# tp7/Sushi

Measured on AMD Instinct MI355X. Metric: subtitle events/sec (matchTemplate+argmax) + max |shift err| vs cv2, 1/2/4/8 GPU, higher is better.
Workload: dtype f32; 1 GPU; BASELINE configs[2] (the north_star target's configuration): 3000 events, 120-min 12000 Hz float32 src/dst, +-120 s window (P=2880001 positions, patterns U[1,5] s), explicit centres; the whole job every step; global_events=3000, sample_type=float32, hard_events=0, events_with_a_planted_answer=3000, method=TM_SQDIFF_NORMED+argmin (what wav.py:185-186 does; see SURVEY F1), kernel_variant=2

## Files before the change

### sushi_amd/csrc/plan_core.hpp

```cpp
#ifndef SUSHI_PLAN_CORE_HPP
#define SUSHI_PLAN_CORE_HPP

#include <limits.h>
#include <math.h>
#include <stdint.h>
#include <stdio.h>
#include <stdlib.h>
#include <string.h>

#include <algorithm>
#include <cmath>
#include <vector>

#include "sushi_geometry.hpp"

namespace sushi {

inline int64_t cand_capacity(int64_t pairs) {
    const int64_t want = pairs * 64;
    return want < (1 << 16) ? (1 << 16) : (want > (1 << 24) ? (1 << 24) : want);
}

struct WsLayout { size_t tspec, y, cand, pair_lb, pairmap, tconst, tiles, candbuf, dummy, slb, acc, plist, slist, citems,
                  tspec_low, ylow, audit_mark, slist2, dense_search, ditems, votes, total; };
// ... 197 lines not shown
            sb.item_count[kern] = mac_items(s, lay, a0, b0, kern, plan.items, &sb.chunk_group[kern]);
        }
        subs.push_back(sb);
        a0 = b0;
    }
    return SUSHI_HIP_OK;
}

inline bool complete_whole_cut(const std::vector<SearchDesc>& descs, Plan& plan) {
    Plan tmp;
    std::vector<SubBatch> subs;
    if (build_plan(descs, search_layouts(descs), plan.ws_whole, tmp, subs) != SUSHI_HIP_OK || subs.empty()) return false;
    if (subs.size() > plan.subs.size()) return false;
    if (tmp.order.size() > plan.order.size() - plan.whole_order_first || tmp.items.size() > plan.whole_items_room) return false;
    std::copy(tmp.order.begin(), tmp.order.end(), plan.order.begin() + (ptrdiff_t)plan.whole_order_first);
    std::copy(tmp.items.begin(), tmp.items.end(), plan.items.begin() + (ptrdiff_t)plan.whole_items_first);
    for (SubBatch& sb : subs) {
        sb.order_first += (int)plan.whole_order_first;
        for (int kern = 0; kern < 2; ++kern) sb.item_first[kern] += (int)(plan.whole_items_first / (1 + MAC_SPW));
    }
    plan.subs_whole.swap(subs);
    plan.whole_pending = false;
    return true;
}

struct BatchLayout { size_t desc, keys, flags, viol, flag_list, subc, tnorm, counters, order, items, ws, total; };

constexpr size_t SUBC_BYTES = 256;
constexpr int SUBC_SCOUNT = 8;
static_assert(sizeof(SubCounters) <= SUBC_SCOUNT * sizeof(int), "the scount words lie behind the SubCounters");
enum ScountSlot {
    SC_SLIST = 0,
    SC_CITEMS = 1,
    SC_ANY_DENSE = 4,
    SC_SLIST2 = 5,
    SC_DENSE_LISTED = 6,
    SC_LIST3 = 7,
    SC_WORDS = 8
};
static_assert((SUBC_SCOUNT + SC_WORDS) * sizeof(int) <= SUBC_BYTES, "the scount words fit the sub-batch's block");
inline BatchLayout batch_layout(int n, int path, size_t n_order_ints, size_t n_item_ints, size_t ws_bytes, size_t n_subs, int64_t total_segs) {
    BatchLayout b;
    size_t o = 0;
    b.desc = o; o += align_up((size_t)n * sizeof(SearchDesc), 256);
    b.order = o; o += path == SUSHI_HIP_PATH_FFT ? align_up(n_order_ints * sizeof(int32_t), 256) : 0;
    b.items = o; o += path == SUSHI_HIP_PATH_FFT ? align_up(n_item_ints * sizeof(int32_t), 256) : 0;
    b.keys = o; o += align_up((size_t)2 * n * sizeof(unsigned long long), 256);
    b.flags = o; o += align_up((size_t)n * sizeof(int), 256);
    b.viol = o; o += align_up((size_t)n * sizeof(int), 256);
    b.flag_list = o; o += align_up((size_t)n * sizeof(int), 256);
    b.subc = o; o += std::max<size_t>(n_subs, 1) * SUBC_BYTES;
    b.tnorm = o; o += align_up((size_t)total_segs * sizeof(float), 256);
    b.counters = o; o += align_up(sizeof(RunCounters), 256);
    b.ws = o; o += path == SUSHI_HIP_PATH_FFT ? align_up(ws_bytes, 256) : 0;
    b.total = o;
    return b;
}

inline int make_descs(const SushiHipRequest* req, int n, int tp, std::vector<SearchDesc>& out, int64_t* n_tiles,
                      int64_t dst_n = INT64_MAX, int64_t src_n = INT64_MAX) {
    out.resize(n);
    int64_t tiles = 0, pairs = 0, segs = 0;
    for (int k = 0; k < n; ++k) {
        const SushiHipRequest& r = req[k];
        if (!request_fits(r, dst_n, src_n)) return SUSHI_HIP_EINVAL;
        SearchDesc d;
// ... 93 lines not shown
```

### sushi_amd/csrc/run_policy.hpp

```cpp
#ifndef SUSHI_RUN_POLICY_HPP
#define SUSHI_RUN_POLICY_HPP

#include <stdint.h>
#include <string.h>

#include <algorithm>

#include "sushi_geometry.hpp"

namespace sushi {

enum RunKind { RUN_ARGMIN, RUN_THRESHOLD, RUN_BEST };

struct Learnt {
    int band = -1;
    int band_decided_method = -1;
    int band_votes[2] = {0, 0};
    int suspended = 0;
    unsigned suspended_at = 0;
    unsigned long long last_transformed = 0;
    void forget() { *this = Learnt(); }
};

struct LastRun {
    RunKind kind = RUN_ARGMIN;
    int band = -1;
    bool whole_cut = false;
    bool suspended = false;
    int64_t direct_pairs = 0;
    bool ran = false;
};

constexpr double SUSPEND_LEFT_SHARE = 0.75;
constexpr unsigned LOOK_AGAIN_MASK = 63u;
constexpr int64_t EXCLUDE_FROM_PAIRS = 3000, EXCLUDE_PAIRS_PER_SEARCH = 2;
constexpr double BAND_VOTE_SHARE = 0.75;
constexpr int64_t DIRECT_SLOTS_MIN = 4096, DIRECT_USUAL_PART = 8;
constexpr int64_t DIRECT_FIRST_RUN_PART = 2;

inline void absorb_counts(Learnt& l, int exclusion, unsigned run_seq, unsigned long long transformed, unsigned long long audited,
                          int64_t plan_pairs) {
// ... 20 lines not shown
    return exclusion == SUSHI_HIP_EXCLUDE_ALWAYS || exclusion == SUSHI_HIP_EXCLUDE_BAND || exclusion == SUSHI_HIP_EXCLUDE_WHOLE ||
           (exclusion == SUSHI_HIP_EXCLUDE_AUTO && !suspended && pairs > EXCLUDE_FROM_PAIRS + EXCLUDE_PAIRS_PER_SEARCH * (int64_t)n_sub);
}

inline bool listed_run_excludes(int exclusion) { return exclusion != SUSHI_HIP_EXCLUDE_NEVER; }

inline bool form_chosen(int exclusion) { return exclusion == SUSHI_HIP_EXCLUDE_BAND || exclusion == SUSHI_HIP_EXCLUDE_WHOLE; }
inline bool vote_due(const Learnt& l, int exclusion, int method) {
    return !form_chosen(exclusion) && (l.band < 0 || l.band_decided_method != method);
}
inline void decide_form(Learnt& l, int method, int looked_at, int with_room) {
    l.band_votes[0] = looked_at; l.band_votes[1] = with_room;
    l.band = l.band_votes[0] > 0 && (double)l.band_votes[1] >= BAND_VOTE_SHARE * (double)l.band_votes[0] ? 1 : 0;
    l.band_decided_method = method;
}
inline int exclusion_form(const Learnt& l, int exclusion) {
    return !form_chosen(exclusion) ? l.band : exclusion == SUSHI_HIP_EXCLUDE_BAND ? 1 : 0;
}

inline int64_t direct_slots(unsigned long long last_transformed, int64_t pairs, int64_t plan_pairs) {
    int64_t direct64 = std::min<int64_t>(pairs, std::max<int64_t>(DIRECT_SLOTS_MIN, pairs / DIRECT_USUAL_PART));
    if ((double)last_transformed * (double)pairs > (double)direct64 * (double)plan_pairs) direct64 = pairs;
    else if (last_transformed == 0) direct64 = std::min<int64_t>(pairs, std::max<int64_t>(DIRECT_SLOTS_MIN, pairs / DIRECT_FIRST_RUN_PART));
    return direct64;
}

enum { PILOT_ROWS_BY_SEARCH = 0, PILOT_ROWS_LIST = 1 };
inline int pilot_rows_route(const char* setting) {
    if (!setting || !*setting || !strcmp(setting, "search")) return PILOT_ROWS_BY_SEARCH;
    return !strcmp(setting, "list") ? PILOT_ROWS_LIST : -1;
}
inline bool pilot_rows_by_search(int route) { return route != PILOT_ROWS_LIST; }

inline void begin_run(LastRun& last, RunKind kind) {
    last = LastRun();
    last.kind = kind; last.ran = true;
}

inline void report_last_run(const LastRun& last, const Learnt& l, const RunCounters& c, SushiHipBatchDiag* diag) {
    const bool argmin = last.kind == RUN_ARGMIN;
    diag->pairs_transformed = (int64_t)c.pairs_transformed + last.direct_pairs;
    diag->band = last.band;
    diag->suspended = argmin && last.suspended ? 1 : 0;
    diag->band_votes[0] = argmin ? l.band_votes[0] : 0; diag->band_votes[1] = argmin ? l.band_votes[1] : 0;
    diag->second_look_audited = argmin ? (int64_t)c.second_look_audited : 0;
}

}
#endif
```

### sushi_amd/csrc/sushi_fft.hip

```cpp

#include <hip/hip_runtime.h>
#include <stdint.h>
#include <float.h>
#include <limits.h>
#include <stdio.h>
#include <stdlib.h>
#include <string.h>

#include <algorithm>
#include <cmath>
#include <memory>
#include <mutex>
#include <new>
#include <string>
#include <type_traits>
#include <vector>

#include "../../include/sushi_hip.h"
#include "sushi_common.hpp"
#include "sushi_internal.hpp"
#include "fft_core.hpp"
#include "mac_core.hpp"
#include "plan_core.hpp"
#include "batch_core.hpp"
// ... 41 lines not shown
        return base + (size_t)k * WORDS;
    }
    void give(unsigned long long* p) {
        if (!p) return;
        std::lock_guard<std::mutex> g(mu);
        free_list.push_back((int)((p - base) / WORDS));
    }
};
static HostSlots g_host_slots;

struct LanePool {
    static constexpr int MAX_DEVICES = 16;
    std::mutex mu;
    hipStream_t st[MAX_DEVICES][MAX_LANES] = {};
    hipStream_t get(int lane) {
        int dev = 0;
        if (hipGetDevice(&dev) != hipSuccess || dev < 0 || dev >= MAX_DEVICES) return nullptr;
        std::lock_guard<std::mutex> g(mu);
        if (!st[dev][lane] && hipStreamCreateWithFlags(&st[dev][lane], hipStreamNonBlocking) != hipSuccess) st[dev][lane] = nullptr;
        return st[dev][lane];
    }
};
static LanePool g_lane_pool;

struct SushiHipBatch {
    const SushiHipStream* dst = nullptr;
    const SushiHipStream* src = nullptr;
    int n = 0, path = 0, variant = 0, method = SUSHI_HIP_METHOD_SQDIFF_NORMED, exclusion = SUSHI_HIP_EXCLUDE_AUTO;
    Learnt learnt;
    LastRun last;
    unsigned run_seq = 0;
    int audit_every = 2;
    int pilot_rows = PILOT_ROWS_BY_SEARCH;
    int bound_model = SUSHI_HIP_BOUND_WORST_CASE;
    BoundFault fault;
    unsigned long long* host_stats = nullptr;
    hipEvent_t stats_ready = nullptr;
    bool stats_pending = false;
    int32_t* packed_out = nullptr;
    int32_t* early_out = nullptr;
    BatchPlanState states[2];
    BatchPlanState *now = &states[0], *spare = &states[1];
    bool planned = false;
    size_t mem_bytes = 0, ws_cap = 0;
    char* mem = nullptr;
    hipStream_t last_stream = nullptr;
    hipEvent_t uploaded = nullptr;
    hipStream_t lane_stream[MAX_LANES] = {};
    hipEvent_t lane_done[MAX_LANES] = {};
    hipEvent_t fork = nullptr;
    void forget_learnt() { learnt.forget(); last = LastRun(); }
    ~SushiHipBatch() {
        for (int l = 1; l < MAX_LANES; ++l) {
            if (lane_stream[l]) (void)hipStreamSynchronize(lane_stream[l]);
            if (lane_done[l]) (void)hipEventDestroy(lane_done[l]);
        }
        if (fork) (void)hipEventDestroy(fork);
        if (uploaded) { (void)hipEventSynchronize(uploaded); (void)hipEventDestroy(uploaded); }
        if (stats_pending && stats_ready) (void)hipEventSynchronize(stats_ready);
        if (stats_ready) (void)hipEventDestroy(stats_ready);
        g_host_slots.give(host_stats);
    }
};

static SubView last_sub(const SushiHipBatch* b) {
    const std::vector<SubBatch>& subs = b->last.whole_cut ? b->now->plan.subs_whole : b->now->plan.subs;
// ... 174 lines not shown
        ma.n_items = sb.item_count[kern];
        const int chunks = (low ? LROWE : ROWE) / MAC_BW;
        ma.chunk_group = std::min(sb.chunk_group[kern], chunks / 8);
        const dim3 grid((unsigned)chunks * (unsigned)ma.n_items);
        auto go = [&](auto row) {
            if (kern == 0) hipLaunchKernelGGL(mac_kernel<decltype(row)::value>, grid, dim3(MAC_THREADS), 0, st, ma);
            else hipLaunchKernelGGL(mac_long_kernel<decltype(row)::value>, grid, dim3(MAC_THREADS), 0, st, ma);
        };
        if (low) go(std::integral_constant<int, LROWE>()); else go(std::integral_constant<int, ROWE>());
        if (launch_ok() != SUSHI_HIP_OK) return SUSHI_HIP_ELAUNCH;
    }
    return SUSHI_HIP_OK;
}

static int launch_mac_list(const RunCtx& c, const SubView& v, hipStream_t st, const int* list, const int* count, int n_list,
                           const int* dense_search, int long_only) {
    MacListArgs la;
    la.dense_search = dense_search; la.long_only = long_only;
    la.spec = (const uint4*)c.dst->spec; la.spec_blocks = c.dst->blocks; la.tspec = (const uint4*)v.tspec; la.y = v.y;
    la.searches = c.searches + v.sb.a0; la.tconst = v.tconst; la.pairmap = v.pairmap; la.list = list; la.count = count;
    la.n_list = n_list; la.sub_first_seg = v.sb.first_seg; la.sub_first_pair = v.sb.first_pair;
    const int64_t want = (int64_t)n_list * MACL_PARTS;
    hipLaunchKernelGGL(mac_list_kernel, dim3((unsigned)std::min<int64_t>(want, 256 * 32)), dim3(MACL_THREADS), 0, st, la);
    return launch_ok();
}

static int launch_mac_rows(const RunCtx& c, const SubView& v, hipStream_t st, const BoundArgs& ba, const int mode) {
    const SubBatch& sb = v.sb;
    MacRowsArgs ra;
    ra.spec = (const uint4*)c.dst->spec; ra.spec_blocks = c.dst->blocks; ra.tspec = (const uint4*)v.tspec; ra.y = v.y;
    ra.searches = c.searches + sb.a0; ra.tconst = v.tconst; ra.mark = ba.audit_mark; ra.n_sub = v.n_sub;
    ra.sub_first_seg = sb.first_seg; ra.sub_first_pair = sb.first_pair; ra.dense_search = v.dense_search;
    ra.plist = ba.plist; ra.first_search = ba.first_search; ra.audit_seq = ba.audit_seq; ra.audit_every = ba.audit_every;
    const int64_t rows_want = (int64_t)v.n_sub * MACL_PARTS;
    const dim3 grid0((unsigned)std::min<int64_t>(rows_want, 256 * 32)), grid1((unsigned)std::min<int64_t>(rows_want, 256 * 16));
    auto go = [&](auto m) {
        if (sb.item_count[0] > 0) hipLaunchKernelGGL((mac_rows_kernel<0, decltype(m)::value>), grid0, dim3(MACL_THREADS), 0, st, ra);
        if (sb.item_count[1] > 0) hipLaunchKernelGGL((mac_rows_kernel<1, decltype(m)::value>), grid1, dim3(MACL_THREADS), 0, st, ra);
    };
    if (mode == ROWS_FIRST) go(std::integral_constant<int, ROWS_FIRST>());
    else if (mode == ROWS_REST) go(std::integral_constant<int, ROWS_REST>());
    else go(std::integral_constant<int, ROWS_MARKED>());
    return launch_ok();
}

static int launch_ifft(const RunCtx& c, const IfftArgs& x, unsigned grid, hipStream_t st) {
    const bool strided = x.count && !x.list_direct;
    return launch_method(c.method, [&](auto m) {
        if (strided) hipLaunchKernelGGL(ifft_list_kernel<decltype(m)::value>, dim3(grid), dim3(FT), 0, st, x);
        else hipLaunchKernelGGL(ifft_kernel<decltype(m)::value>, dim3(grid), dim3(FT), 0, st, x);
    });
}

static int bound_pairs(const RunCtx& c, const SubView& v, hipStream_t st, const int band, BoundArgs& ba) {
    const SubBatch& sb = v.sb;
    ba = bound_args(c, v);
    ba.band = band;
    ba.y = band ? (const uint2*)v.ylow : (const uint2*)v.y;
    if (!band && hipMemsetAsync(ba.acc, 0, (size_t)sb.pairs * 2 * sizeof(float), st) != hipSuccess) return SUSHI_HIP_ELAUNCH;
    const int per_pair = band ? 1 : 16;
    const int64_t want = (sb.pairs * per_pair + BOUND_THREADS / 64 - 1) / (BOUND_THREADS / 64);
    const unsigned grid = (unsigned)std::min<int64_t>(want, 256 * (band ? 3 * (c.lanes > 1 ? 2 : 4) : 4));
    auto go = [&](auto energies) {
        if (band) hipLaunchKernelGGL(bound_low_kernel<decltype(energies)::value>, dim3(grid), dim3(BOUND_THREADS), 0, st, ba);
        else hipLaunchKernelGGL(bound_kernel<decltype(energies)::value>, dim3(grid), dim3(BOUND_THREADS), 0, st, ba);
    };
    if (ba.worst_case) go(std::false_type()); else go(std::true_type());
    if (launch_ok() != SUSHI_HIP_OK || launch_slb(c, v, ba, st) != SUSHI_HIP_OK) return SUSHI_HIP_ELAUNCH;
    if (c.b->fault.period > 0) return launch_bound_fault(c, v, st);
    return SUSHI_HIP_OK;
}

static int second_look(const RunCtx& c, const SubView& v, hipStream_t st, BoundArgs& ba) {
    ba.list = ba.slist; ba.list_count = ba.scount;
    ba.list2 = v.slist2; ba.list2_count = v.n_slist2;
    hipLaunchKernelGGL(bound_low_exact_kernel, dim3(256 * 4), dim3(BLE_T), 0, st, ba);
    if (launch_ok() != SUSHI_HIP_OK) return SUSHI_HIP_ELAUNCH;
    if (launch_method(c.method, [&](auto m) { hipLaunchKernelGGL(slb_list_kernel<decltype(m)::value>, dim3(256 * 2), dim3(256), 0, st, ba); }) !=
        SUSHI_HIP_OK)
        return SUSHI_HIP_ELAUNCH;
    if (c.b->fault.period > 0 && launch_bound_fault(c, v, st) != SUSHI_HIP_OK) return SUSHI_HIP_ELAUNCH;
    hipLaunchKernelGGL(survivor2_kernel, dim3(256), dim3(256), 0, st, ba);
    return launch_ok();
}

static int exclude_pairs(const RunCtx& c, const SubView& v, hipStream_t st, const int band, IfftArgs& ip, hipEvent_t& t0) {
    const SubBatch& sb = v.sb;
    BoundArgs ba;
    if (bound_pairs(c, v, st, band, ba) != SUSHI_HIP_OK) return SUSHI_HIP_ELAUNCH;
    prof_end(c.pc, t0, SUSHI_HIP_STAGE_BOUND, st);
    t0 = prof_begin(c.pc, st);
    hipLaunchKernelGGL(pilot_kernel, dim3((unsigned)v.n_sub), dim3(64), 0, st, ba);
    if (launch_ok() != SUSHI_HIP_OK) return SUSHI_HIP_ELAUNCH;
    ip.slb = ba.slb; ip.audit_mark = nullptr;
    ip.order = ba.plist; ip.count = nullptr;
    const bool by_search = pilot_rows_by_search(c.b->pilot_rows);
    if (band && by_search && launch_mac_rows(c, v, st, ba, ROWS_FIRST) != SUSHI_HIP_OK) return SUSHI_HIP_ELAUNCH;
    if (band && launch_mac_list(c, v, st, ba.plist, nullptr, v.n_sub, nullptr, by_search ? 1 : 0) != SUSHI_HIP_OK) return SUSHI_HIP_ELAUNCH;
    if (launch_ifft(c, ip, (unsigned)v.n_sub, st) != SUSHI_HIP_OK) return SUSHI_HIP_ELAUNCH;
    hipLaunchKernelGGL(survivor_kernel, dim3((unsigned)((sb.pairs + 255) / 256)), dim3(256), 0, st, ba);
    if (launch_ok() != SUSHI_HIP_OK) return SUSHI_HIP_ELAUNCH;
    ip.order = ba.slist; ip.count = ba.scount; ip.audit_mark = ba.audit_mark;
    if (!band) return SUSHI_HIP_OK;
    if (second_look(c, v, st, ba) != SUSHI_HIP_OK) return SUSHI_HIP_ELAUNCH;
    ip.order = ba.list2; ip.count = ba.list2_count;
    hipLaunchKernelGGL(dense_search_kernel, dim3((unsigned)v.n_sub), dim3(64), 0, st, ba, v.dense_search, v.n_dense_listed);
    const size_t second = (size_t)(sb.item_first[1] - sb.item_first[0]) * (1 + MAC_SPW);
    hipLaunchKernelGGL(dense_repack_kernel, dim3(2), dim3(REPACK_THREADS), 0, st, v.items, sb.item_count[0], v.items + second,
                       sb.item_count[1], v.dense_search, v.n_sub, v.ditems, v.ditems + second, v.n_dense_listed, (int)(sb.pairs / 8),
                       v.any_dense);
    if (launch_ok() != SUSHI_HIP_OK) return SUSHI_HIP_ELAUNCH;
    if (launch_mac_rows(c, v, st, ba, by_search ? ROWS_REST : ROWS_MARKED) != SUSHI_HIP_OK) return SUSHI_HIP_ELAUNCH;
    if (sb.long_patterns && launch_mac_list(c, v, st, ba.list2, ba.list2_count, (int)sb.pairs, v.dense_search, 1) != SUSHI_HIP_OK) return SUSHI_HIP_ELAUNCH;
    return launch_mac(c, v, st, false, v.any_dense, v.ditems);
}

static int transform_listed(const RunCtx& c, const SubView& v, hipStream_t st, IfftArgs ip) {
    const SubBatch& sb = v.sb;
    const SushiHipBatch* b = c.b;
    const unsigned direct = (unsigned)direct_slots(b->learnt.last_transformed, sb.pairs, b->now->plan.pairs);
    ip.list_first = 0; ip.list_direct = 1;
    if (launch_ifft(c, ip, direct, st) != SUSHI_HIP_OK) return SUSHI_HIP_ELAUNCH;
    if ((int64_t)direct >= sb.pairs) return SUSHI_HIP_OK;
    ip.list_first = (int)direct; ip.list_direct = 0;
    return launch_ifft(c, ip, (unsigned)std::min<int64_t>(sb.pairs - direct, 1024), st);
}

static int stage_refine(const RunCtx& c, const SubView& v, hipStream_t st) {
    hipEvent_t t0 = prof_begin(c.pc, st);
    RefineParams rp;
    rp.r = c.r; rp.searches = c.searches; rp.first_search = v.sb.a0; rp.n_sub = v.n_sub; rp.sub_first_pair = v.sb.first_pair;
    rp.cand = v.cand; rp.pair_lb = v.pair_lb; rp.gkeys = c.gkeys; rp.keys = c.keys; rp.flags = c.flags; rp.flag_list = c.flag_list + v.sb.a0;
    rp.sub = v.sub; rp.counters = c.counters; rp.delta = (float)c.delta; rp.method = c.method; rp.citems = v.citems; rp.n_citems = v.n_citems;
    rp.viol = c.viol; rp.early = reinterpret_cast<int4*>(c.b->early_out);
    const int rc = launch_refine(rp, st);
    if (rc == SUSHI_HIP_OK) prof_end(c.pc, t0, SUSHI_HIP_STAGE_REFINE, st);
    return rc;
}

static int stage_collect(const RunCtx& c, const SubView& v, hipStream_t st, IfftArgs ia) {
    hipEvent_t t0 = prof_begin(c.pc, st);
    ia.citems = v.citems; ia.n_citems = v.n_citems;
    if (launch_method(c.method, [&](auto m) { hipLaunchKernelGGL(collect_kernel<decltype(m)::value>, dim3(COLLECT_GRID), dim3(FT), 0, st, ia); }) !=
        SUSHI_HIP_OK)
        return SUSHI_HIP_ELAUNCH;
// ... 235 lines not shown
    return total;
}, 0, 0); }

static int plan_and_upload(SushiHipBatch* b, const SushiHipRequest* req_host, int n, hipStream_t st) {
    const BatchSpec spec{b->path, direct_variant_tile(b->variant), b->ws_cap, b->mem_bytes, b->dst->n, b->src->n, b->dst->dtype == SUSHI_HIP_F32 ? 4.0 : 1.0};
    const int rc = stage_batch(req_host, n, spec, getenv("SUSHI_HIP_LANES"), g_plan_cache, *b->spare);
    if (rc != SUSHI_HIP_OK) return rc;
    if (b->uploaded ? hipEventSynchronize(b->uploaded) != hipSuccess : hipEventCreateWithFlags(&b->uploaded, hipEventDisableTiming) != hipSuccess)
        return SUSHI_HIP_ELAUNCH;
    std::swap(b->now, b->spare);
    b->forget_learnt();
    b->planned = hipMemcpyAsync(b->mem + b->now->lay.desc, b->now->upload.data(), b->now->upload.size(), hipMemcpyHostToDevice, st) == hipSuccess &&
                 hipEventRecord(b->uploaded, st) == hipSuccess;
    return b->planned ? SUSHI_HIP_OK : SUSHI_HIP_ELAUNCH;
}

int sushi_hip_batch_create(const SushiHipStream* dst, const SushiHipStream* src, const SushiHipRequest* req_host, int n,
                           int path, int variant, size_t workspace_cap_bytes, void* mem_dev, size_t mem_bytes,
                           void* hip_stream, SushiHipBatch** out) { return c_boundary([&]() -> int {
    if (!dst || !src || !req_host || !mem_dev || !out || n <= 0) return SUSHI_HIP_EINVAL;
    if (path != SUSHI_HIP_PATH_FFT && path != SUSHI_HIP_PATH_DIRECT) return SUSHI_HIP_EINVAL;
    if (dst->dtype != src->dtype) return SUSHI_HIP_EINVAL;
    if ((uintptr_t)mem_dev & 255) return SUSHI_HIP_EALIGN;
    if (path == SUSHI_HIP_PATH_FFT && !dst->spec) return SUSHI_HIP_EINVAL;
    if ((variant = variant_of(path, variant, req_host, n)) < 0) return SUSHI_HIP_EINVAL;
    SushiHipBatch* b = new (std::nothrow) SushiHipBatch();
    if (!b) return SUSHI_HIP_ENOMEM;
    std::unique_ptr<SushiHipBatch> guard(b);
    b->dst = dst; b->src = src; b->n = n; b->path = path; b->variant = variant;
    b->mem = (char*)mem_dev; b->mem_bytes = mem_bytes; b->ws_cap = workspace_cap_bytes;
    const char* e = getenv("SUSHI_HIP_AUDIT_EVERY");
    if (e && *e) { const int v = atoi(e); b->audit_every = v < 0 ? 0 : v; }
    if ((b->pilot_rows = pilot_rows_route(getenv("SUSHI_HIP_PILOT_ROWS"))) < 0) return SUSHI_HIP_EINVAL;
    const char* m = getenv("SUSHI_HIP_BOUND_MODEL");
    if (m && !strcmp(m, "statistical")) b->bound_model = SUSHI_HIP_BOUND_STATISTICAL;
    const char* f = getenv("SUSHI_HIP_TEST_BOUND_FAULT");
    if (f && *f && !parse_bound_fault(f, &b->fault)) return SUSHI_HIP_EINVAL;
    const int rc = plan_and_upload(b, req_host, n, (hipStream_t)hip_stream);
    if (rc != SUSHI_HIP_OK) return rc;
    *out = guard.release();
    return SUSHI_HIP_OK;
}); }

int sushi_hip_batch_reset(SushiHipBatch* b, const SushiHipRequest* req_host, int n, void* hip_stream) { return c_boundary([&]() -> int {
    if (!b || !req_host || n != b->n) return SUSHI_HIP_EINVAL;
    if (b->stats_pending && b->stats_ready) { (void)hipEventSynchronize(b->stats_ready); b->stats_pending = false; }
    return plan_and_upload(b, req_host, n, (hipStream_t)hip_stream);
}); }

int sushi_hip_batch_info(const SushiHipBatch* b, SushiHipBatchInfo* info) {
    if (!b || !info) return SUSHI_HIP_EINVAL;
    memset(info, 0, sizeof(*info));
    info->n_search = b->n; info->path = b->path; info->variant = b->variant;
    info->sub_batches = b->path == SUSHI_HIP_PATH_FFT ? (int32_t)b->now->plan.subs.size() : 1;
    info->direct_tiles = b->now->n_tiles;
    info->fft_pairs = b->now->plan.pairs; info->fft_segments = b->now->plan.segs;
    info->workspace_bytes = b->now->plan.ws_bytes; info->mem_bytes = b->now->lay.total;
    info->flops = b->now->flops; info->algorithmic_bytes = b->now->algorithmic_bytes;
    info->lanes = b->path == SUSHI_HIP_PATH_FFT ? b->now->plan.lanes : 1;
    return SUSHI_HIP_OK;
}

void sushi_hip_batch_destroy(SushiHipBatch* b) { delete b; }

int sushi_hip_batch_set_method(SushiHipBatch* b, int method) {
    if (!b) return SUSHI_HIP_EINVAL;
// ... 198 lines not shown
```

### sushi_amd/csrc/sushi_fft_bound.inc

```

struct BoundArgs {
    const uint2* y;
    const double* dst_stats;
    const SearchDesc* searches;
    int sub_first_pair;
    int first_search;
    int64_t dst_len;
    const int* pairmap;
    const TemplConsts* tconst;
    const double* ubase;
    const double* sbase;
    int64_t nb;
    const double* coarse;
    int64_t nc;
    float* slb;
    float* acc;
    int n_sub;
    int n_pairs;
    int* plist;
    int* slist;
    int* scount;
    const int* order;
    const unsigned long long* gkeys;
    float* pair_lb;
// ... 338 lines not shown
    const int lane = threadIdx.x & 63;
    int base = 0;
    if (lane == 0 && m) {
        base = atomicAdd(count, __popcll(m));
        atomicAdd(&counters->pairs_transformed, (unsigned long long)__popcll(m));
    }
    base = __shfl(base, 0, 64);
    if (add) list[base + __popcll(m & ((1ull << lane) - 1ull))] = pr;
}

__global__ __launch_bounds__(256)
void survivor_kernel(BoundArgs a) {
    const int b = blockIdx.x * 256 + threadIdx.x;
    bool keep = false;
    int pr = 0;
    if (b < a.n_pairs) {
        pr = a.order[b];
        const int k = a.pairmap[pr];
        bool audit = false;
        if (a.plist[k] != pr) {
            const bool excluded = bound_excludes(a.slb, pr, a.gkeys[a.first_search + k]);
            if (excluded && audited_search(a, k)) {
                const SearchDesc sd = a.searches[k];
                audit = audit_pair_of(a, sd, k) == a.sub_first_pair + pr - sd.first_pair;
            }
            if (excluded && !audit) a.pair_lb[pr] = __builtin_inff();
            keep = !excluded || audit;
        }
        if (a.audit_mark) a.audit_mark[pr] = (audit ? MARK_AUDITED : 0) | (keep ? MARK_LISTED : 0);
    }
    append_pairs(a.slist, a.scount, a.counters, keep, pr);
}

enum { ROWS_MARKED = 0, ROWS_FIRST = 1, ROWS_REST = 2 };
struct MacRowsArgs {
    const uint4* spec;
    int64_t spec_blocks;
    const uint4* tspec;
    uint4* y;
    const SearchDesc* searches;
    const TemplConsts* tconst;
    const unsigned char* mark;
    int n_sub;
    int sub_first_seg;
    int sub_first_pair;
    const int* dense_search;
    const int* plist;
    int first_search;
    unsigned audit_seq;
    int audit_every;
};
template <int SMAX>
__device__ __forceinline__ void mac_row_of_pair(const MacRowsArgs& a, const FftLayout& lay, const sushi_mac::h8 (&tt)[SMAX],
                                                const uint4* __restrict__ zsp, const int p0, const int ip, const float sy, const int e,
                                                const int z_zero) {
    typedef _Float16 h2 __attribute__((ext_vector_type(2)));
    const long long I = lay.pair0 + ip;
    sushi_mac::acc4 acc = sushi_mac::zero_acc();
#pragma unroll
    for (int s6 = 0; s6 < SMAX; s6 += 6) {
        sushi_mac::h8 z[6];
#pragma unroll
        for (int t = 0; t < 6; ++t) {
            const long long jj = s6 + t < lay.n_seg ? FFT_STEP * I + s6 + t : (long long)z_zero;
            z[t] = as_h8(zsp[(size_t)(jj < z_zero ? jj : z_zero) * ROWE]);
        }
#pragma unroll
        for (int t = 0; t < 6; ++t) {
            const sushi_mac::zrow zr = {z[t], sushi_mac::rot_mi(z[t])};
            sushi_mac::mac4(acc, tt[s6 + t], zr);
        }
    }
    unsigned o[sushi_mac::BINS];
#pragma unroll
    for (int q = 0; q < sushi_mac::BINS; ++q) {
        const h2 h = {(_Float16)(acc.re[q] * sy), (_Float16)(acc.im[q] * sy)};
        o[q] = __builtin_bit_cast(unsigned, h);
    }
    a.y[(size_t)(p0 + ip) * ROWE + e] = uint4{o[0], o[1], o[2], o[3]};
}
template <int SMAX, int MODE>
__device__ __forceinline__ void mac_rows_of_search(const MacRowsArgs& a, const SearchDesc& sd, const FftLayout& lay, const int k,
                                                   const float sy, const int e, unsigned long long (*masks)[4], const int z_zero) {
// ... 4 lines not shown
    int audit = -1;
    if (MODE != ROWS_MARKED && audited_search(a, k)) audit = audit_pair_of(a, sd, k);
    if (MODE == ROWS_REST) {
        bool any = false;
        for (int i = tid; i < lay.n_pairs; i += MACL_THREADS) any = any || (i != audit && (a.mark[p0 + i] & MARK_LISTED));
        if (!__syncthreads_or(any)) return;
    }
    sushi_mac::h8 tt[SMAX];
#pragma unroll
    for (int s = 0; s < SMAX; ++s) tt[s] = s < lay.n_seg ? as_h8(tsp[(size_t)s * ROWE]) : sushi_mac::zero_h8();
    if (MODE == ROWS_FIRST) {
        const int pilot = a.plist[k] - p0;
        mac_row_of_pair<SMAX>(a, lay, tt, zsp, p0, pilot, sy, e, z_zero);
        if (audit >= 0 && audit < lay.n_pairs && audit != pilot) mac_row_of_pair<SMAX>(a, lay, tt, zsp, p0, audit, sy, e, z_zero);
        return;
    }
    for (int base = 0; base < lay.n_pairs; base += MACL_THREADS) {
        __syncthreads();
        const int i = base + tid;
        const bool on = i < lay.n_pairs && (MODE == ROWS_MARKED || i != audit) && (a.mark[p0 + i] & MARK_LISTED);
        const unsigned long long bm = __ballot(on);
        if ((tid & 63) == 0) (*masks)[tid >> 6] = bm;
        __syncthreads();
        for (int w = 0; w < 4; ++w) {
            unsigned long long m = (*masks)[w];
            while (m) {
                const int bit = __builtin_ctzll(m);
                m &= m - 1;
                mac_row_of_pair<SMAX>(a, lay, tt, zsp, p0, base + 64 * w + bit, sy, e, z_zero);
            }
        }
    }
}
template <int LONG, int MODE>
__global__ __launch_bounds__(MACL_THREADS)
void mac_rows_kernel(MacRowsArgs a) {
    __shared__ unsigned long long masks[4];
    const int z_zero = (int)(a.spec_blocks < 0x7fffffff ? a.spec_blocks : 0x7fffffff);
    for (long long it = blockIdx.x; it < (long long)a.n_sub * MACL_PARTS; it += gridDim.x) {
        const int k = (int)(it / MACL_PARTS);
        if (MODE != ROWS_FIRST && a.dense_search[k]) continue;
        const int e = (int)(it % MACL_PARTS) * MACL_THREADS + threadIdx.x;
        const SearchDesc sd = a.searches[k];
        const FftLayout lay = fft_layout(sd.win_start, sd.n_pos, sd.tmpl_len);
        const float sy = a.tconst[k].mac_scale;
        if (LONG) {
            if (lay.n_seg > MAC_SMAX_SHORT && lay.n_seg <= MAC_SMAX_LONG) mac_rows_of_search<MAC_SMAX_LONG, MODE>(a, sd, lay, k, sy, e, &masks, z_zero);
        } else {
            if (lay.n_seg <= 6) mac_rows_of_search<6, MODE>(a, sd, lay, k, sy, e, &masks, z_zero);
            else if (lay.n_seg <= 12) mac_rows_of_search<12, MODE>(a, sd, lay, k, sy, e, &masks, z_zero);
            else if (lay.n_seg <= MAC_SMAX_SHORT) mac_rows_of_search<MAC_SMAX_SHORT, MODE>(a, sd, lay, k, sy, e, &masks, z_zero);
        }
    }
}

constexpr int BLE_LOGN = 13;
constexpr int BLE_N = sushi_fft::Plan<BLE_LOGN>::N, BLE_T = sushi_fft::Plan<BLE_LOGN>::NT;
static_assert(BLE_N == FN / 2, "the low band sampled at every second position");
__global__ __launch_bounds__(BLE_T)
void bound_low_exact_kernel(BoundArgs a) {
    __shared__ __attribute__((aligned(16))) float lds[sushi_fft::lds_floats<BLE_LOGN>()];
    __shared__ unsigned red[BLE_T / 64];
    typedef _Float16 h2 __attribute__((ext_vector_type(2)));
    const int n = *a.list_count;
    if (n > a.n_pairs / 5) return;
    for (int slot = blockIdx.x; slot < n; slot += gridDim.x) {
        int tid = threadIdx.x;
        asm volatile("" : "+v"(tid));
        const sushi_fft::Twiddles tw = sushi_fft::load_twiddles<BLE_LOGN, 1>(tid, twiddles());
        const int pr = a.list[slot];
        const uint32_t* __restrict__ row = reinterpret_cast<const uint32_t*>(a.y) + (size_t)pr * (LROWE * 4);
// ... 35 lines not shown
        const int slot = base + threadIdx.x;
        bool keep = false;
        int pr = 0;
        if (slot < n) {
            pr = a.list[slot];
            keep = true;
            if (second_look && !(a.audit_mark[pr] & MARK_AUDITED)) {
                const int k = a.pairmap[pr];
                if (bound_excludes(a.slb, pr, a.gkeys[a.first_search + k])) {
                    const unsigned h = ((unsigned)(a.sub_first_pair + pr) * 2654435761u + a.audit_seq * 40503u) >> 11;
                    if (a.audit_every > 0 && h % (16u * (unsigned)a.audit_every) == 0u) {
                        a.audit_mark[pr] = MARK_AUDITED | MARK_LISTED | MARK_SECOND_LOOK;
                    } else {
                        keep = false;
                        a.pair_lb[pr] = __builtin_inff();
                        a.audit_mark[pr] = 0;
                    }
                }
            }
        }
        const unsigned long long m = __ballot(keep), act = __ballot(slot < n);
        const int lane = threadIdx.x & 63;
        const int dropped = __popcll(act) - __popcll(m);
        int b0 = 0;
        if (lane == 0 && m) b0 = atomicAdd(a.list2_count, __popcll(m));
        if (lane == 0 && dropped > 0)
            atomicAdd(&a.counters->pairs_transformed, (unsigned long long)0 - (unsigned long long)dropped);
        b0 = __shfl(b0, 0, 64);
        if (keep) a.list2[b0 + __popcll(m & ((1ull << lane) - 1ull))] = pr;
    }
}

__global__ __launch_bounds__(64)
void dense_search_kernel(BoundArgs a, int* __restrict__ dense_search, int* __restrict__ any) {
    const int lane = threadIdx.x;
    const int k = blockIdx.x;
    const SearchDesc sd = a.searches[k];
    const FftLayout lay = fft_layout(sd.win_start, sd.n_pos, sd.tmpl_len);
    const int p0 = first_pair_in_sub(a.sub_first_pair, sd);
    int listed = 0;
    for (int i = lane; i < lay.n_pairs; i += 64) listed += (a.audit_mark[p0 + i] & MARK_LISTED) ? 1 : 0;
#pragma unroll
    for (int d = 32; d >= 1; d >>= 1) listed += __shfl_xor(listed, d, 64);
    if (lane == 0) {
        const int dense = listed * 5 > lay.n_pairs * 2 ? 1 : 0;
        dense_search[k] = dense;
        if (dense) atomicAdd(any, listed);
    }
}

constexpr int REPACK_THREADS = 1024;
__global__ __launch_bounds__(REPACK_THREADS)
void dense_repack_kernel(const int* __restrict__ items0, int n_items0, const int* __restrict__ items1, int n_items1,
                         int* __restrict__ dense_search, int n_search, int* __restrict__ out0, int* __restrict__ out1,
                         const int* __restrict__ listed_dense, int min_listed, int* __restrict__ any) {
    if (*listed_dense < min_listed) {
        if (blockIdx.x == 0) for (int k = threadIdx.x; k < n_search; k += REPACK_THREADS) dense_search[k] = 0;
        return;
    }
    if (threadIdx.x == 0) *any = 1;
    const int* __restrict__ items = blockIdx.x == 0 ? items0 : items1;
    const int n_items = blockIdx.x == 0 ? n_items0 : n_items1;
    int* __restrict__ out = blockIdx.x == 0 ? out0 : out1;
    if (n_items == 0) return;
    __shared__ int wave_tot[REPACK_THREADS / 64];
    __shared__ int carry_s, out_base_s;
    const int tid = threadIdx.x, lane = tid & 63, wave = tid >> 6;
    for (int e = tid; e < n_items * (1 + MAC_SPW); e += REPACK_THREADS) out[e] = -1;
    if (tid == 0) out_base_s = 0;
    __syncthreads();
    const int n_ent = n_items * MAC_SPW;
    for (int c = 0; c < MAC_CLASSES; ++c) {
        if (tid == 0) carry_s = 0;
        __syncthreads();
// ... 28 lines not shown
```

### sushi_amd/csrc/sushi_fft_plan.inc

```

template <typename F> int launch_method(int method, F&& f) {
    if (method == SUSHI_HIP_METHOD_CCOEFF_NORMED) f(std::integral_constant<int, SUSHI_HIP_METHOD_CCOEFF_NORMED>());
    else f(std::integral_constant<int, SUSHI_HIP_METHOD_SQDIFF_NORMED>());
    return launch_ok();
}
template <typename F> int launch_dtype(int dtype, F&& f) {
    if (dtype == SUSHI_HIP_F32) f((float*)nullptr);
    else f((uint8_t*)nullptr);
    return launch_ok();
}

struct ProfSpan { hipEvent_t t0, t1; int stage; };
struct ProfCall { std::vector<ProfSpan> spans; };
bool g_prof_on = false;
std::vector<ProfCall> g_prof;

inline hipEvent_t prof_begin(ProfCall* pc, hipStream_t st) {
    if (!pc) return nullptr;
    hipEvent_t e = nullptr;
    if (hipEventCreate(&e) != hipSuccess) return nullptr;
    (void)hipEventRecord(e, st);
    return e;
}
inline void prof_end(ProfCall* pc, hipEvent_t t0, int stage, hipStream_t st) {
    if (!pc || !t0) return;
    hipEvent_t e = nullptr;
    if (hipEventCreate(&e) != hipSuccess) return;
    (void)hipEventRecord(e, st);
    pc->spans.push_back(ProfSpan{t0, e, stage});
}

struct SubView {
    const SubBatch& sb;
    int n_sub;
    uint32_t* tspec; uint4 *y, *tspec_low, *ylow, *dummy; unsigned long long* cand; TemplConsts* tconst; TileDesc* tiles; int32_t* candbuf;
    float *pair_lb, *slb, *acc, *tnorm_rest; unsigned char* audit_mark; SubCounters* sub; const int32_t *order, *items;
    int *pairmap, *plist, *slist, *slist2, *votes, *dense_search, *ditems, *citems;
    int *n_slist, *n_citems, *any_dense, *n_slist2, *n_dense_listed, *n_list3;
    SubView(char* mem, const BatchLayout& lay, size_t ws_lane, const SubBatch& s, size_t si) : sb(s), n_sub(s.b0 - s.a0) {
        const WsLayout w = ws_layout(s.pairs, s.segs, n_sub);
        char* p = mem + lay.ws + (size_t)s.lane * ws_lane;
        tspec = (uint32_t*)(p + w.tspec); y = (uint4*)(p + w.y); tspec_low = (uint4*)(p + w.tspec_low); ylow = (uint4*)(p + w.ylow); dummy = (uint4*)(p + w.dummy);
        cand = (unsigned long long*)(p + w.cand); tconst = (TemplConsts*)(p + w.tconst); tiles = (TileDesc*)(p + w.tiles); candbuf = (int32_t*)(p + w.candbuf);
        pair_lb = (float*)(p + w.pair_lb); slb = (float*)(p + w.slb); acc = (float*)(p + w.acc); tnorm_rest = (float*)(mem + lay.tnorm) + s.first_seg;
        audit_mark = (unsigned char*)(p + w.audit_mark); sub = (SubCounters*)(mem + lay.subc + si * SUBC_BYTES);
        int* const scount = (int*)sub + SUBC_SCOUNT;
        n_slist = scount + SC_SLIST; n_citems = scount + SC_CITEMS; any_dense = scount + SC_ANY_DENSE; n_slist2 = scount + SC_SLIST2;
        n_dense_listed = scount + SC_DENSE_LISTED; n_list3 = scount + SC_LIST3;
        order = (const int32_t*)(mem + lay.order) + s.order_first;
        items = (const int32_t*)(mem + lay.items) + (size_t)s.item_first[0] * (1 + MAC_SPW);
        pairmap = (int*)(p + w.pairmap); plist = (int*)(p + w.plist); slist = (int*)(p + w.slist); slist2 = (int*)(p + w.slist2);
        votes = (int*)(p + w.votes); dense_search = (int*)(p + w.dense_search); ditems = (int*)(p + w.ditems); citems = (int*)(p + w.citems);
    }
};
```

Before: 374,700 events/s.

## Split rest-row MAC work into fixed-size pair items instead of per-search blocks

```diff
diff --git a/sushi_amd/csrc/plan_core.hpp b/sushi_amd/csrc/plan_core.hpp
--- a/sushi_amd/csrc/plan_core.hpp
+++ b/sushi_amd/csrc/plan_core.hpp
@@ -253,6 +253,7 @@
 enum ScountSlot {
     SC_SLIST = 0,
     SC_CITEMS = 1,
+    SC_REST_ITEMS = 2,
     SC_ANY_DENSE = 4,
     SC_SLIST2 = 5,
     SC_DENSE_LISTED = 6,
diff --git a/sushi_amd/csrc/run_policy.hpp b/sushi_amd/csrc/run_policy.hpp
--- a/sushi_amd/csrc/run_policy.hpp
+++ b/sushi_amd/csrc/run_policy.hpp
@@ -7,6 +7,14 @@
 #include <algorithm>
 
 #include "sushi_geometry.hpp"
+
+#ifndef SUSHI_HHD
+#ifdef __HIPCC__
+#define SUSHI_HHD __host__ __device__ inline
+#else
+#define SUSHI_HHD inline
+#endif
+#endif
 
 namespace sushi {
 
@@ -93,6 +101,32 @@
 }
 inline bool pilot_rows_by_search(int route) { return route != PILOT_ROWS_LIST; }
 
+enum { REST_ROWS_BY_ITEM = 0, REST_ROWS_BY_SEARCH = 1 };
+inline int rest_rows_route(const char* setting) {
+    if (!setting || !*setting || !strcmp(setting, "items")) return REST_ROWS_BY_ITEM;
+    return !strcmp(setting, "search") ? REST_ROWS_BY_SEARCH : -1;
+}
+inline bool rest_rows_by_item(int route) { return route != REST_ROWS_BY_SEARCH; }
+
+#ifndef SUSHI_REST_ITEM_PAIRS
+#define SUSHI_REST_ITEM_PAIRS 4
+#endif
+constexpr int REST_ITEM_PAIRS = SUSHI_REST_ITEM_PAIRS;
+static_assert(REST_ITEM_PAIRS >= 1, "an item holds a pair");
+SUSHI_HHD bool rest_pair_to_form(int listed, int i, int audit) { return listed != 0 && i != audit; }
+SUSHI_HHD unsigned long long rest_item_starts(unsigned long long form, int before, int per_item) {
+    unsigned long long starts = 0;
+    int rank = before;
+    for (unsigned long long m = form; m; m &= m - 1, ++rank)
+        if (rank % per_item == 0) starts |= m & (~m + 1);
+    return starts;
+}
+SUSHI_HHD unsigned long long rest_item_take(unsigned long long form, int room) {
+    unsigned long long take = 0;
+    for (unsigned long long m = form; m && room > 0; m &= m - 1, --room) take |= m & (~m + 1);
+    return take;
+}
+
 inline void begin_run(LastRun& last, RunKind kind) {
     last = LastRun();
     last.kind = kind; last.ran = true;
diff --git a/sushi_amd/csrc/sushi_fft.hip b/sushi_amd/csrc/sushi_fft.hip
--- a/sushi_amd/csrc/sushi_fft.hip
+++ b/sushi_amd/csrc/sushi_fft.hip
@@ -97,6 +97,7 @@
     unsigned run_seq = 0;
     int audit_every = 2;
     int pilot_rows = PILOT_ROWS_BY_SEARCH;
+    int rest_rows = REST_ROWS_BY_ITEM;
     int bound_model = SUSHI_HIP_BOUND_WORST_CASE;
     BoundFault fault;
     unsigned long long* host_stats = nullptr;
@@ -337,7 +338,8 @@
     ra.searches = c.searches + sb.a0; ra.tconst = v.tconst; ra.mark = ba.audit_mark; ra.n_sub = v.n_sub;
     ra.sub_first_seg = sb.first_seg; ra.sub_first_pair = sb.first_pair; ra.dense_search = v.dense_search;
     ra.plist = ba.plist; ra.first_search = ba.first_search; ra.audit_seq = ba.audit_seq; ra.audit_every = ba.audit_every;
-    const int64_t rows_want = (int64_t)v.n_sub * MACL_PARTS;
+    ra.items = v.slist; ra.item_count = v.n_rest_items; ra.pairmap = v.pairmap; ra.n_pairs = (int)sb.pairs;
+    const int64_t rows_want = (int64_t)(mode == ROWS_ITEMS ? sb.pairs : v.n_sub) * MACL_PARTS;
     const dim3 grid0((unsigned)std::min<int64_t>(rows_want, 256 * 32)), grid1((unsigned)std::min<int64_t>(rows_want, 256 * 16));
     auto go = [&](auto m) {
         if (sb.item_count[0] > 0) hipLaunchKernelGGL((mac_rows_kernel<0, decltype(m)::value>), grid0, dim3(MACL_THREADS), 0, st, ra);
@@ -345,6 +347,7 @@
     };
     if (mode == ROWS_FIRST) go(std::integral_constant<int, ROWS_FIRST>());
     else if (mode == ROWS_REST) go(std::integral_constant<int, ROWS_REST>());
+    else if (mode == ROWS_ITEMS) go(std::integral_constant<int, ROWS_ITEMS>());
     else go(std::integral_constant<int, ROWS_MARKED>());
     return launch_ok();
 }
@@ -409,13 +412,15 @@
     if (!band) return SUSHI_HIP_OK;
     if (second_look(c, v, st, ba) != SUSHI_HIP_OK) return SUSHI_HIP_ELAUNCH;
     ip.order = ba.list2; ip.count = ba.list2_count;
-    hipLaunchKernelGGL(dense_search_kernel, dim3((unsigned)v.n_sub), dim3(64), 0, st, ba, v.dense_search, v.n_dense_listed);
+    const bool by_item = by_search && rest_rows_by_item(c.b->rest_rows);
+    hipLaunchKernelGGL(dense_search_kernel, dim3((unsigned)v.n_sub), dim3(64), 0, st, ba, v.dense_search, v.n_dense_listed,
+                       by_item ? v.slist : nullptr, v.n_rest_items);
     const size_t second = (size_t)(sb.item_first[1] - sb.item_first[0]) * (1 + MAC_SPW);
     hipLaunchKernelGGL(dense_repack_kernel, dim3(2), dim3(REPACK_THREADS), 0, st, v.items, sb.item_count[0], v.items + second,
                        sb.item_count[1], v.dense_search, v.n_sub, v.ditems, v.ditems + second, v.n_dense_listed, (int)(sb.pairs / 8),
                        v.any_dense);
     if (launch_ok() != SUSHI_HIP_OK) return SUSHI_HIP_ELAUNCH;
-    if (launch_mac_rows(c, v, st, ba, by_search ? ROWS_REST : ROWS_MARKED) != SUSHI_HIP_OK) return SUSHI_HIP_ELAUNCH;
+    if (launch_mac_rows(c, v, st, ba, by_item ? ROWS_ITEMS : by_search ? ROWS_REST : ROWS_MARKED) != SUSHI_HIP_OK) return SUSHI_HIP_ELAUNCH;
     if (sb.long_patterns && launch_mac_list(c, v, st, ba.list2, ba.list2_count, (int)sb.pairs, v.dense_search, 1) != SUSHI_HIP_OK) return SUSHI_HIP_ELAUNCH;
     return launch_mac(c, v, st, false, v.any_dense, v.ditems);
 }
@@ -717,6 +722,7 @@
     const char* e = getenv("SUSHI_HIP_AUDIT_EVERY");
     if (e && *e) { const int v = atoi(e); b->audit_every = v < 0 ? 0 : v; }
     if ((b->pilot_rows = pilot_rows_route(getenv("SUSHI_HIP_PILOT_ROWS"))) < 0) return SUSHI_HIP_EINVAL;
+    if ((b->rest_rows = rest_rows_route(getenv("SUSHI_HIP_REST_ROWS"))) < 0) return SUSHI_HIP_EINVAL;
     const char* m = getenv("SUSHI_HIP_BOUND_MODEL");
     if (m && !strcmp(m, "statistical")) b->bound_model = SUSHI_HIP_BOUND_STATISTICAL;
     const char* f = getenv("SUSHI_HIP_TEST_BOUND_FAULT");
diff --git a/sushi_amd/csrc/sushi_fft_bound.inc b/sushi_amd/csrc/sushi_fft_bound.inc
--- a/sushi_amd/csrc/sushi_fft_bound.inc
+++ b/sushi_amd/csrc/sushi_fft_bound.inc
@@ -394,7 +394,7 @@
     append_pairs(a.slist, a.scount, a.counters, keep, pr);
 }
 
-enum { ROWS_MARKED = 0, ROWS_FIRST = 1, ROWS_REST = 2 };
+enum { ROWS_MARKED = 0, ROWS_FIRST = 1, ROWS_REST = 2, ROWS_ITEMS = 3 };
 struct MacRowsArgs {
     const uint4* spec;
     int64_t spec_blocks;
@@ -411,6 +411,10 @@
     int first_search;
     unsigned audit_seq;
     int audit_every;
+    const int* items;
+    const int* item_count;
+    const int* pairmap;
+    int n_pairs;
 };
 template <int SMAX>
 __device__ __forceinline__ void mac_row_of_pair(const MacRowsArgs& a, const FftLayout& lay, const sushi_mac::h8 (&tt)[SMAX],
@@ -481,11 +485,58 @@
         }
     }
 }
+template <int SMAX>
+__device__ __forceinline__ void mac_rows_of_item(const MacRowsArgs& a, const SearchDesc& sd, const FftLayout& lay, const int k,
+                                                 const float sy, const int e, const int z_zero, const int first) {
+    const uint4* __restrict__ tsp = a.tspec + (size_t)(sd.first_seg - a.sub_first_seg) * ROWE + e;
+    const uint4* __restrict__ zsp = a.spec + e;
+    const int p0 = first_pair_in_sub(a.sub_first_pair, sd);
+    const int audit = audited_search(a, k) ? audit_pair_of(a, sd, k) : -1;
+    sushi_mac::h8 tt[SMAX];
+#pragma unroll
+    for (int s = 0; s < SMAX; ++s) tt[s] = s < lay.n_seg ? as_h8(tsp[(size_t)s * ROWE]) : sushi_mac::zero_h8();
+    int room = REST_ITEM_PAIRS;
+    for (int base = first; base < lay.n_pairs && room > 0; base += 64) {
+        const int i = base + (threadIdx.x & 63);
+        const bool on = i < lay.n_pairs && rest_pair_to_form(a.mark[p0 + i] & MARK_LISTED, i, audit);
+        unsigned long long m = rest_item_take(__ballot(on), room);
+        room -= __popcll(m);
+        while (m) {
+            const int bit = __builtin_ctzll(m);
+            m &= m - 1;
+            mac_row_of_pair<SMAX>(a, lay, tt, zsp, p0, base + bit, sy, e, z_zero);
+        }
+    }
+}
 template <int LONG, int MODE>
 __global__ __launch_bounds__(MACL_THREADS)
 void mac_rows_kernel(MacRowsArgs a) {
     __shared__ unsigned long long masks[4];
     const int z_zero = (int)(a.spec_blocks < 0x7fffffff ? a.spec_blocks : 0x7fffffff);
+    if (MODE == ROWS_ITEMS) {
+        const int listed = *a.item_count;
+        const int n_items = listed < a.n_pairs ? listed : a.n_pairs;
+        for (long long it = blockIdx.x; it < (long long)n_items * MACL_PARTS; it += gridDim.x) {
+            const int first = __builtin_amdgcn_readfirstlane(a.items[it / MACL_PARTS]);
+            if ((unsigned)first >= (unsigned)a.n_pairs) continue;
+            const int k = __builtin_amdgcn_readfirstlane(a.pairmap[first]);
+            if ((unsigned)k >= (unsigned)a.n_sub || a.dense_search[k]) continue;
+            const int e = (int)(it % MACL_PARTS) * MACL_THREADS + threadIdx.x;
+            const SearchDesc sd = a.searches[k];
+            const FftLayout lay = fft_layout(sd.win_start, sd.n_pos, sd.tmpl_len);
+            const float sy = a.tconst[k].mac_scale;
+            const int i0 = first - first_pair_in_sub(a.sub_first_pair, sd);
+            if ((unsigned)i0 >= (unsigned)lay.n_pairs) continue;
+            if (LONG) {
+                if (lay.n_seg > MAC_SMAX_SHORT && lay.n_seg <= MAC_SMAX_LONG) mac_rows_of_item<MAC_SMAX_LONG>(a, sd, lay, k, sy, e, z_zero, i0);
+            } else {
+                if (lay.n_seg <= 6) mac_rows_of_item<6>(a, sd, lay, k, sy, e, z_zero, i0);
+                else if (lay.n_seg <= 12) mac_rows_of_item<12>(a, sd, lay, k, sy, e, z_zero, i0);
+                else if (lay.n_seg <= MAC_SMAX_SHORT) mac_rows_of_item<MAC_SMAX_SHORT>(a, sd, lay, k, sy, e, z_zero, i0);
+            }
+        }
+        return;
+    }
     for (long long it = blockIdx.x; it < (long long)a.n_sub * MACL_PARTS; it += gridDim.x) {
         const int k = (int)(it / MACL_PARTS);
         if (MODE != ROWS_FIRST && a.dense_search[k]) continue;
@@ -587,14 +638,31 @@
 }
 
 __global__ __launch_bounds__(64)
-void dense_search_kernel(BoundArgs a, int* __restrict__ dense_search, int* __restrict__ any) {
+void dense_search_kernel(BoundArgs a, int* __restrict__ dense_search, int* __restrict__ any, int* __restrict__ items,
+                         int* __restrict__ item_count) {
     const int lane = threadIdx.x;
     const int k = blockIdx.x;
     const SearchDesc sd = a.searches[k];
     const FftLayout lay = fft_layout(sd.win_start, sd.n_pos, sd.tmpl_len);
     const int p0 = first_pair_in_sub(a.sub_first_pair, sd);
-    int listed = 0;
-    for (int i = lane; i < lay.n_pairs; i += 64) listed += (a.audit_mark[p0 + i] & MARK_LISTED) ? 1 : 0;
+    const int audit = items && audited_search(a, k) ? audit_pair_of(a, sd, k) : -1;
+    int listed = 0, formed = 0;
+    for (int base = 0; base < lay.n_pairs; base += 64) {
+        const int i = base + lane;
+        const int on = i < lay.n_pairs ? (a.audit_mark[p0 + i] & MARK_LISTED) : 0;
+        listed += on ? 1 : 0;
+        if (items) {
+            const unsigned long long form = __ballot(rest_pair_to_form(on, i, audit));
+            const unsigned long long starts = rest_item_starts(form, formed, REST_ITEM_PAIRS);
+            formed += __popcll(form);
+            if (starts) {
+                int slot = 0;
+                if (lane == 0) slot = atomicAdd(item_count, __popcll(starts));
+                slot = __shfl(slot, 0, 64) + __popcll(starts & ((1ull << lane) - 1ull));
+                if (((starts >> lane) & 1ull) && slot < a.n_pairs) items[slot] = p0 + i;
+            }
+        }
+    }
 #pragma unroll
     for (int d = 32; d >= 1; d >>= 1) listed += __shfl_xor(listed, d, 64);
     if (lane == 0) {
diff --git a/sushi_amd/csrc/sushi_fft_plan.inc b/sushi_amd/csrc/sushi_fft_plan.inc
--- a/sushi_amd/csrc/sushi_fft_plan.inc
+++ b/sushi_amd/csrc/sushi_fft_plan.inc
@@ -36,7 +36,7 @@
     uint32_t* tspec; uint4 *y, *tspec_low, *ylow, *dummy; unsigned long long* cand; TemplConsts* tconst; TileDesc* tiles; int32_t* candbuf;
     float *pair_lb, *slb, *acc, *tnorm_rest; unsigned char* audit_mark; SubCounters* sub; const int32_t *order, *items;
     int *pairmap, *plist, *slist, *slist2, *votes, *dense_search, *ditems, *citems;
-    int *n_slist, *n_citems, *any_dense, *n_slist2, *n_dense_listed, *n_list3;
+    int *n_slist, *n_citems, *any_dense, *n_slist2, *n_dense_listed, *n_list3, *n_rest_items;
     SubView(char* mem, const BatchLayout& lay, size_t ws_lane, const SubBatch& s, size_t si) : sb(s), n_sub(s.b0 - s.a0) {
         const WsLayout w = ws_layout(s.pairs, s.segs, n_sub);
         char* p = mem + lay.ws + (size_t)s.lane * ws_lane;
@@ -46,7 +46,7 @@
         audit_mark = (unsigned char*)(p + w.audit_mark); sub = (SubCounters*)(mem + lay.subc + si * SUBC_BYTES);
         int* const scount = (int*)sub + SUBC_SCOUNT;
         n_slist = scount + SC_SLIST; n_citems = scount + SC_CITEMS; any_dense = scount + SC_ANY_DENSE; n_slist2 = scount + SC_SLIST2;
-        n_dense_listed = scount + SC_DENSE_LISTED; n_list3 = scount + SC_LIST3;
+        n_dense_listed = scount + SC_DENSE_LISTED; n_list3 = scount + SC_LIST3; n_rest_items = scount + SC_REST_ITEMS;
         order = (const int32_t*)(mem + lay.order) + s.order_first;
         items = (const int32_t*)(mem + lay.items) + (size_t)s.item_first[0] * (1 + MAC_SPW);
         pairmap = (int*)(p + w.pairmap); plist = (int*)(p + w.plist); slist = (int*)(p + w.slist); slist2 = (int*)(p + w.slist2);
```

New measurement: 384,500 events/s, median of 6. +2.6%, better.
